# cr1m5onk1ng/text_similarity

Measured on AMD Instinct MI355X. Metric: sentences/sec encoded + Mpairs/sec cosine top-k @ N=1M d=384, higher is better.
Workload: dtype bf16 encoder / f16 selection / fp32 scores

## Files before the change

include/tsim.h:

```cpp
#ifndef TSIM_H
#define TSIM_H

#include <stddef.h>
#include <stdint.h>

#ifdef __cplusplus
extern "C" {
#endif

#define TSIM_OK 0
#define TSIM_EINVAL 1
#define TSIM_EHIP 2
#define TSIM_ENOMEM 3
#define TSIM_EUNSUPPORTED 4

#define TSIM_F32 0
#define TSIM_BF16 1

#define TSIM_ARCH_BERT 0
#define TSIM_ARCH_MPNET 1
#define TSIM_ARCH_ROBERTA 2

int tsim_version(void);
const char *tsim_last_error(void);
// ... 201 lines not shown
    int32_t dense_act;
    int32_t normalize;
} tsim_sentence_head;

int tsim_encoder_forward_head(tsim_encoder *enc, const int32_t *tok_ids, const int32_t *tok_type, const int32_t *tok_pos,
                              const int32_t *tok_col, const int32_t *cu_seqlens, int32_t T, int32_t B, int32_t max_len,
                              const tsim_sentence_head *head, float *emb_f32, void *unit_f16, int ld_unit,
                              float *unit_rho_max, void *last_hidden_bf16, void *stream);

int tsim_encoder_forward_spans(tsim_encoder *enc, const int32_t *tok_ids, const int32_t *tok_type, const int32_t *tok_pos,
                               const int32_t *tok_col, const int32_t *cu_seqlens, int32_t T, int32_t B, int32_t max_len,
                               float *pooled_f32, void *unit_f16, int ld_unit, float *unit_rho_max,
                               void *last_hidden_bf16, float *logits_f32, const int32_t *span_seq, const int32_t *span_cu,
                               const int32_t *span_tok, int32_t S, int32_t n_span_tok, float *span_out_f32,
                               void *span_unit_f16, int ld_span_unit, float *span_rho_max, void *stream);

#define TSIM_ENC_ERR_TOKEN_ID 1
#define TSIM_ENC_ERR_POSITION 2
#define TSIM_ENC_ERR_MAX_LEN 4
#define TSIM_ENC_ERR_TOKEN_TYPE 8
#define TSIM_ENC_ERR_SPAN 16
int tsim_encoder_error_flags(tsim_encoder *enc, int32_t *flags_host, void *stream);

int tsim_wordpiece_create(const char *vocab_text, const int64_t *vocab_offsets, int32_t vocab_size,
                          const char *continuing_prefix, int32_t unk_id, const int32_t *prefix_ids, int32_t n_prefix,
                          const int32_t *suffix_ids, int32_t n_suffix, int32_t lowercase, int32_t max_input_chars_per_word,
                          const char *added_text, const int64_t *added_offsets, int32_t n_added, void **handle);
void tsim_wordpiece_destroy(void *handle);
int tsim_wordpiece_encode(void *handle, const char *text, const int64_t *text_offsets, int64_t n, int32_t max_len,
                          int32_t n_threads, int32_t *out_ids, int64_t out_capacity, int32_t *out_lens, uint8_t *handled);

#ifdef __cplusplus
}
#endif
#endif
```

text_similarity_amd/_lib.py:

```python
from __future__ import annotations

import ctypes as C
import os

_HERE = os.path.dirname(os.path.abspath(__file__))
LIB_PATH = os.environ.get("TSIM_LIB") or os.path.join(_HERE, "libtsim.so")

TSIM_F32, TSIM_BF16 = 0, 1
TSIM_I32, TSIM_I64 = 2, 3
LIST_ST_ROW, LIST_ST_LIMS = 1, 2
ARCH_BERT, ARCH_MPNET, ARCH_ROBERTA = 0, 1, 2
W_BF16, W_MXFP8 = 0, 1
POOL_MEAN, POOL_CLS, POOL_MAX, POOL_MEAN_SQRT_LEN = 0, 1, 2, 3
ACT_IDENTITY, ACT_TANH, ACT_RELU = 0, 1, 2
SPACE_COSINE, SPACE_DOT, SPACE_L2 = 0, 1, 2
ENC_ERR_SPAN = 16
RANGE_SLOT_CAP = 2048
RANGE_MERGE_MAX_LISTS = 64


class TsimError(RuntimeError):
    pass


# ... 104 lines not shown
    "tsim_time_next_topk": (None, [C.c_void_p, C.c_void_p]),
    "tsim_topk_merge": (C.c_int, [C.c_void_p, C.c_void_p, C.c_int, C.c_int64, C.c_int, C.c_int, C.c_void_p,
                                  C.c_void_p, C.c_void_p]),
    "tsim_topk_merge_strided": (C.c_int, [C.c_void_p, C.c_void_p, C.c_int, C.c_int64, C.c_int, C.c_int, C.c_int64, C.c_int64,
                                          C.c_void_p, C.c_void_p, C.c_void_p]),
    "tsim_wordpiece_create": (C.c_int, [C.c_char_p, C.c_void_p, C.c_int32, C.c_char_p, C.c_int32, C.c_void_p, C.c_int32, C.c_void_p,
                                        C.c_int32, C.c_int32, C.c_int32, C.c_char_p, C.c_void_p, C.c_int32, C.POINTER(C.c_void_p)]),
    "tsim_wordpiece_destroy": (None, [C.c_void_p]),
    "tsim_wordpiece_encode": (C.c_int, [C.c_void_p, C.c_char_p, C.c_void_p, C.c_int64, C.c_int32, C.c_int32, C.c_void_p, C.c_int64,
                                        C.c_void_p, C.c_void_p]),
    "tsim_cos_sim": (C.c_int, [C.c_void_p, C.c_int64, C.c_void_p, C.c_int64, C.c_int, C.c_void_p, C.c_void_p]),
    "tsim_mean_pool": (C.c_int, [C.c_void_p, C.c_int, C.c_void_p, C.c_int64, C.c_int, C.c_int, C.c_void_p,
                                 C.c_void_p]),
    "tsim_pool": (C.c_int, [C.c_void_p, C.c_int, C.c_void_p, C.c_int64, C.c_int, C.c_int, C.c_int, C.c_void_p, C.c_void_p]),
    "tsim_dense_rows": (C.c_int, [C.c_void_p, C.c_int64, C.c_int, C.c_void_p, C.c_void_p, C.c_int, C.c_int, C.c_int, C.c_void_p,
                                  C.c_void_p]),
    "tsim_quantize_mxfp8": (C.c_int, [C.c_void_p, C.c_int64, C.c_int, C.c_void_p, C.c_void_p, C.c_void_p]),
    "tsim_gemm_mxfp8": (C.c_int, [C.c_void_p, C.c_void_p, C.c_void_p, C.c_void_p, C.c_void_p, C.c_void_p, C.c_int, C.c_int,
                                  C.c_int, C.c_void_p]),
    "tsim_encoder_create": (C.c_int, [C.POINTER(EncoderConfigC), C.POINTER(EncoderWeightsC),
                                      C.POINTER(C.c_void_p)]),
    "tsim_encoder_destroy": (None, [C.c_void_p]),
    "tsim_encoder_error_flags": (C.c_int, [C.c_void_p, C.POINTER(C.c_int32), C.c_void_p]),
    "tsim_encoder_forward": (C.c_int, [C.c_void_p, C.c_void_p, C.c_void_p, C.c_void_p, C.c_void_p, C.c_int32,
                                       C.c_int32, C.c_int32, C.c_void_p, C.c_void_p, C.c_int, C.c_void_p, C.c_void_p,
                                       C.c_void_p]),
    "tsim_encoder_set_token_types": (C.c_int, [C.c_void_p, C.c_void_p, C.c_int32]),
    "tsim_encoder_set_cls_head": (C.c_int, [C.c_void_p, C.c_void_p, C.c_void_p, C.c_void_p, C.c_void_p, C.c_int32]),
    "tsim_encoder_set_cls_head_act": (C.c_int, [C.c_void_p, C.c_void_p, C.c_void_p, C.c_void_p, C.c_void_p, C.c_int32, C.c_int32]),
    "tsim_encoder_forward_ex": (C.c_int, [C.c_void_p, C.c_void_p, C.c_void_p, C.c_void_p, C.c_void_p, C.c_void_p, C.c_int32,
                                          C.c_int32, C.c_int32, C.c_void_p, C.c_void_p, C.c_int, C.c_void_p, C.c_void_p,
                                          C.c_void_p, C.c_void_p]),
    "tsim_encoder_forward_head": (C.c_int, [C.c_void_p, C.c_void_p, C.c_void_p, C.c_void_p, C.c_void_p, C.c_void_p, C.c_int32,
                                            C.c_int32, C.c_int32, C.POINTER(SentenceHeadC), C.c_void_p, C.c_void_p, C.c_int,
                                            C.c_void_p, C.c_void_p, C.c_void_p]),
    "tsim_encoder_forward_spans": (C.c_int, [C.c_void_p, C.c_void_p, C.c_void_p, C.c_void_p, C.c_void_p, C.c_void_p, C.c_int32,
                                             C.c_int32, C.c_int32, C.c_void_p, C.c_void_p, C.c_int, C.c_void_p, C.c_void_p,
                                             C.c_void_p, C.c_void_p, C.c_void_p, C.c_void_p, C.c_int32, C.c_int32, C.c_void_p,
                                             C.c_void_p, C.c_int, C.c_void_p, C.c_void_p]),
}

DECLARED_SYMBOLS = tuple(_SIGS)


def lib() -> C.CDLL:
    global _lib
# ... 25 lines not shown
```

text_similarity_amd/build.py:

```python
from __future__ import annotations

import os
import subprocess
import sys
from concurrent.futures import ThreadPoolExecutor

HERE = os.path.dirname(os.path.abspath(__file__))
CSRC = os.path.join(HERE, "csrc")
TAG = os.environ.get("TSIM_BUILD_TAG", "")
OBJ = os.path.join(CSRC, "_obj" + ("_" + TAG if TAG else ""))
LIB = os.path.join(HERE, "libtsim" + ("_" + TAG if TAG else "") + ".so")
SOURCES = ["common.hip", "search.hip", "k1_kl16.hip", "k1_d384.hip", "k1_kl32.hip", "k1_collect.hip", "gemm_pp.hip", "encoder.hip",
           "wordpiece.cpp"]
HOT_KERNELS = ("l2_rows_kernel", "l2_query_rows_kernel", "l2_negate_scores", "flag_all_kernel", "cos_topk_partial", "cos_topk_finalize", "gemm_bf16", "gemm_xres", "ln_rows_gemm", "ln_tail_gemm", "gemm_pp", "attention_kernel",
               "pool_packed_kernel", "dense_rows_kernel", "widen_finalize", "bf_partial", "bf_merge",
               "topk_merge_large", "list_prep", "list_partial", "list_merge", "range_setup", "range_finalize", "range_bf", "range_fill", "range_merge", "span_pool_kernel",
               "pack_sign_rows", "hamming_partial", "hamming_merge", "sign_rescore",
               "embed_ln_kernel", "cls_head_kernel", "cls_head_wide_kernel")
FLAGS = ["--offload-arch=gfx950", "-O3", "-std=c++17", "-fPIC", "-fno-gpu-rdc", "-Wall", "-Wno-unused-function",
         "-I" + os.path.join(os.path.dirname(HERE), "include")]


def _newer(a, bs):
    return os.path.exists(a) and all(os.path.getmtime(a) >= os.path.getmtime(b) for b in bs)


DIAGNOSTIC_DEFINES = ("TSIM_LN_DIAG", "TSIM_X2_DIAG", "TSIM_FF_DIAG", "TSIM_K1_NOSEL", "TSIM_PP_STAMPS", "TSIM_K1_DIAG",
                      "TSIM_ATT_DIAG", "TSIM_L_DIAG")


def build(force: bool = False, verbose: bool = True, extra_flags=(), only=None) -> str:
    bad = [f for f in extra_flags if f.startswith("-D") and ("DIAG" in f or any(d in f for d in DIAGNOSTIC_DEFINES))]
    if bad and not TAG:
        raise RuntimeError(f"{bad}: diagnostic defines produce wrong results; they are refused for the product library — "
                           "set TSIM_BUILD_TAG=<tag> to build libtsim_<tag>.so beside it")
    os.makedirs(OBJ, exist_ok=True)
    hdrs = [os.path.join(CSRC, f) for f in os.listdir(CSRC) if f.endswith(".h")]
# ... 65 lines not shown
```

text_similarity_amd/csrc/encoder.hip:

```cpp
#include <math.h>
#include <cmath>

#include <stdlib.h>
#include <string.h>

#include <vector>

#include <type_traits>
#include <utility>

#include "common.h"
#include "gemm_pp.h"

namespace tsim {

__device__ __forceinline__ int64_t packed_off(int64_t t, int f, int W) {
    return ((t >> 5) * (W >> 3) + (f >> 3)) * 256 + (t & 31) * 8 + (f & 7);
}
__device__ __forceinline__ int64_t group_off(int64_t t, int g, int W, int packed) {
    return packed ? packed_off(t, 8 * g, W) * 2 : (t * W + 8 * g) * 2;
}

template <int VPL, bool TYPED = false>
__global__ __launch_bounds__(256) void embed_ln_kernel(const int32_t *__restrict__ ids,
// ... 736 lines not shown
    for (int t = 0; t < 12; ++t) {
        uint32_t pk[8];
#pragma unroll
        for (int gq = 0; gq < 4; ++gq) {
            const int n = 32 * t + 8 * gq + 4 * h;
            const f32x4 gv = *reinterpret_cast<const f32x4 *>(gamma + n), bv = *reinterpret_cast<const f32x4 *>(beta + n);
            const float o0 = fmaf((acc[t][4 * gq + 0] - mean) * rstd, gv[0], bv[0]);
            const float o1 = fmaf((acc[t][4 * gq + 1] - mean) * rstd, gv[1], bv[1]);
            const float o2 = fmaf((acc[t][4 * gq + 2] - mean) * rstd, gv[2], bv[2]);
            const float o3 = fmaf((acc[t][4 * gq + 3] - mean) * rstd, gv[3], bv[3]);
            pk[2 * gq] = pack_bf16x2(o0, o1);
            pk[2 * gq + 1] = pack_bf16x2(o2, o3);
        }
#pragma unroll
        for (int gq = 0; gq < 4; gq += 2) {
            auto s0 = __builtin_amdgcn_permlane32_swap(pk[2 * gq], pk[2 * gq + 2], false, false);
            auto s1w = __builtin_amdgcn_permlane32_swap(pk[2 * gq + 1], pk[2 * gq + 3], false, false);
            if (live)
                *reinterpret_cast<uint4 *>(reinterpret_cast<char *>(out) + (oo + (4 * t + gq) * ogs)) = make_uint4(s0[0], s1w[0], s0[1], s1w[1]);
        }
    }
}

template <int DH, bool REL, bool PK = false>
__global__ __launch_bounds__(256) __attribute__((amdgpu_waves_per_eu(DH <= 32 ? 6 : 4))) void attention_kernel(const bf16_t *__restrict__ qkv,
                                                        const int32_t *__restrict__ cu, const int32_t *__restrict__ col,
                                                        const float *__restrict__ relb, int relw, int H,
                                                        int heads, float scale, bf16_t *__restrict__ ctx, int B, int xcd_map) {
    constexpr int KS = DH / 16;
    constexpr int OT = (DH + 31) / 32;
    constexpr int ROWB = DH * 2 < 64 ? 64 : DH * 2;
    __shared__ __attribute__((aligned(16))) char vimg[4 * 32 * ROWB];
    typedef __attribute__((ext_vector_type(4))) short s16x4;
    const int lane = threadIdx.x & 63;
    const int wave = __builtin_amdgcn_readfirstlane(threadIdx.x >> 6);
    int seq = blockIdx.x;
    if (xcd_map) {
        seq = (blockIdx.x & 7) * (gridDim.x >> 3) + (blockIdx.x >> 3);
        if (seq >= B) return;
    }
    const int head = blockIdx.y * 4 + wave, qb = blockIdx.z;
    const int t0 = cu[seq], S = cu[seq + 1] - t0;
    if (qb * 32 >= S || head >= heads) return;
    const int r = lane & 31, h = lane >> 5;
    const int64_t H3 = 3 * (int64_t)H;
    const int qi = qb * 32 + r;
// ... 902 lines not shown
                           K, xpacked ? 1 : 0, rpk);
    TSIM_HIP_CHECK(hipGetLastError());
    hipLaunchKernelGGL(ln_split_finish_kernel, dim3((unsigned)nb), dim3(256), 0, st, im, gamma, beta, eps, out, M, opk);
    TSIM_HIP_CHECK(hipGetLastError());
    return TSIM_OK;
}

template <int NW, int NST>
static int ln_rows_gemm(const bf16_t *X, const bf16_t *Wimg32, const float *bias, const bf16_t *res, const float *gamma,
                        const float *beta, float eps, bf16_t *out, int M, int K, hipStream_t st, bool xpacked, bool respacked, bool opacked) {
    constexpr int lds = NST * (NW * 32 * LR_BK * 2 + LR_WBYTES);
    static_assert(lds <= 160 * 1024, "LDS budget");
    auto kern = ln_rows_gemm_kernel<NW, NST>;
    static DevOnce lds_once;
    TSIM_MAX_LDS(lds_once, kern, lds);
    if (K % LR_BK != 0 || K < NST * LR_BK) return fail(TSIM_EUNSUPPORTED, "ln_rows_gemm: K=%d", K);
    if (((int64_t)M + 256) * 768 >= (1ll << 32)) return fail(TSIM_EUNSUPPORTED, "ln_rows_gemm: %d rows of 384 exceed 4 GiB", M);
    hipLaunchKernelGGL(kern, dim3((unsigned)((M + NW * 32 - 1) / (NW * 32))), dim3(NW * 64), lds, st, X, Wimg32, bias, res, gamma,
                       beta, eps, out, M, K, xpacked ? 1 : 0, respacked ? 1 : 0, opacked ? 1 : 0);
    TSIM_HIP_CHECK(hipGetLastError());
    return TSIM_OK;
}

static bool use_packed_layout(int H, int F) {
    return H == 384 && (3 * H) % X2_BN == 0 && F % X2_BN == 0 && F <= 2048;
}

template <int EPI>
static int gemm_plain(const bf16_t *X, const bf16_t *W, const bf16_t *Wp, const float *bias, bf16_t *out, int M, int N,
                      int K, hipStream_t st) {
    if (K == 384 && N % XR_BN == 0) return gemm_xres2<EPI, false>(X, W, bias, out, M, N, st);
    if (K >= 768 && gemm_pp_supported(N, K))
        return gemm_pp(EPI == EPI_GELU ? PP_EPI_GELU : PP_EPI_BIAS, X, Wp ? Wp : W, Wp != nullptr, bias, out, M, N, K, st);
    if (N % 128 == 0)
        return launch_gemm<128, 128, 64, 2, 2, EPI>(X, W, bias, nullptr, nullptr, nullptr, 0.f, out, M, N, K, st);
    return launch_gemm<128, 64, 64, 2, 2, EPI>(X, W, bias, nullptr, nullptr, nullptr, 0.f, out, M, N, K, st);
}

static int gemm_res_ln(const bf16_t *X, const bf16_t *W, const bf16_t *Wp, const float *bias, const bf16_t *res,
                       const float *gamma, const float *beta, float eps, bf16_t *out, int M, int N, int K, float *ybuf,
                       hipStream_t st, const bf16_t *Wimg = nullptr, const bf16_t *Wimg32 = nullptr, bool xpacked = false,
                       float *lnimg = nullptr, bool respacked = false, bool opacked = false) {
    if ((xpacked || respacked || opacked) && N != 384) return fail(TSIM_EINVAL, "gemm_res_ln: the packed layouts are a hidden-384 form");
    if (ybuf && N >= 512 && N % 256 == 0 && gemm_pp_supported(N, K)) {
        int rc = gemm_pp(PP_EPI_F32, X, Wp ? Wp : W, Wp != nullptr, bias, ybuf, M, N, K, st);
        if (rc) return rc;
        return res_ln_rows(ybuf, res, gamma, beta, eps, out, nullptr, nullptr, M, N, st);
    }
    switch (N) {
        case 384: {
            bool after_rows = false;
            if (Wimg32) {
                const int t256 = M / 256;
                const int use = (t256 % 256) >= 128 ? t256 : (t256 / 256) * 256;
                if (use > 0) {
                    int rc = ln_rows_gemm<8, 3>(X, Wimg32, bias, res, gamma, beta, eps, out, use * 256, K, st, xpacked, respacked, opacked);
                    const int m1 = use * 256;
                    if (rc || m1 == M) return rc;
                    X += (int64_t)m1 * K; res += (int64_t)m1 * N; out += (int64_t)m1 * N; M -= m1;
                    after_rows = true;
                }
                if (M <= LS_MAX_BLOCKS * 32 && K % (16 * LT_PF) == 0)
                    return ln_tail_gemm(X, Wimg32, bias, res, gamma, beta, eps, out, M, K, st, xpacked, lnimg, respacked, opacked);
            }
            const int mt = (M + 127) / 128, full = (mt / 256) * 256, rem = mt - full;
            auto main_launch = [&](int rows) {
                return launch_gemm<128, 384, 64, 2, 4, EPI_RES_LN>(X, W, bias, res, gamma, beta, eps, out, rows, N, K, st, Wimg, xpacked, respacked, opacked);
            };
            if (rem > 0 && rem <= 96 && (full > 0 || after_rows)) {
                const int m_main = full * 128;
                if (full > 0) {
                    int rc = main_launch(m_main);
                    if (rc) return rc;
                }
                return launch_gemm<64, 384, 64, 2, 4, EPI_RES_LN>(X + (int64_t)m_main * K, W, bias, res + (int64_t)m_main * N,
                                                                  gamma, beta, eps, out + (int64_t)m_main * N, M - m_main, N, K, st, Wimg, xpacked, respacked, opacked);
            }
            return main_launch(M);
        }
        case 768: return launch_gemm<64, 768, 32, 1, 8, EPI_RES_LN>(X, W, bias, res, gamma, beta, eps, out, M, N, K, st);
        case 64: return launch_gemm<128, 64, 64, 4, 2, EPI_RES_LN>(X, W, bias, res, gamma, beta, eps, out, M, N, K, st);
        default: return fail(TSIM_EUNSUPPORTED, "encoder: hidden size %d has no fused LayerNorm GEMM (64, 384, 768)", N);
    }
}

}

extern "C" int tsim_encoder_create(const tsim_encoder_config *cfg, const tsim_encoder_weights_host *w,
                                   tsim_encoder **out) {
    TSIM_REQUIRE(cfg && w && out, "encoder_create: null pointer");
    const int H = cfg->hidden, F = cfg->ffn, L = cfg->num_layers;
    TSIM_REQUIRE(H == 64 || H == 384 || H == 768 || H == 1024, "encoder_create: hidden=%d unsupported (64, 384, 768, 1024)", H);
    TSIM_REQUIRE(cfg->heads > 0 && H % cfg->heads == 0, "encoder_create: heads=%d does not divide hidden=%d", cfg->heads, H);
    const int dh = H / cfg->heads;
    TSIM_REQUIRE(dh == 16 || dh == 32 || dh == 64, "encoder_create: head_dim=%d unsupported (16, 32, 64)", dh);
    TSIM_REQUIRE(F % 64 == 0 && L > 0 && cfg->max_tokens > 0 && cfg->max_seqs > 0, "encoder_create: bad ffn/layers/capacity");
    TSIM_REQUIRE(cfg->arch == TSIM_ARCH_BERT || cfg->arch == TSIM_ARCH_MPNET || cfg->arch == TSIM_ARCH_ROBERTA, "encoder_create: unknown arch");
    TSIM_REQUIRE(w->word_emb && w->pos_emb && w->emb_ln_g && w->emb_ln_b && w->layers, "encoder_create: missing weights");
    TSIM_REQUIRE(cfg->arch != TSIM_ARCH_MPNET || w->rel_bias, "encoder_create: MPNet needs rel_bias");
    const bool mx = cfg->weight_dtype == TSIM_W_MXFP8;
    TSIM_REQUIRE(cfg->weight_dtype == TSIM_W_BF16 || mx, "encoder_create: unknown weight_dtype %d", cfg->weight_dtype);
    if (mx && !(gemm_pp_mx_supported(H, H) && gemm_pp_mx_supported(3 * H, H) && gemm_pp_mx_supported(F, H) && gemm_pp_mx_supported(H, F)))
        return fail(TSIM_EUNSUPPORTED, "encoder_create: MXFP8 projections need hidden and ffn to be multiples of 256 (got %d, %d)", H, F);
    tsim_encoder *e = new tsim_encoder();
    e->cfg = *cfg;
    e->Tp = (cfg->max_tokens + 127) / 128 * 128 + 128;
    int rc = TSIM_OK;
    auto bail = [&](int code) {
// ... 210 lines not shown
    hipStream_t st = reinterpret_cast<hipStream_t>(stream);
    const tsim_encoder_config &c = e->cfg;
    const int H = c.hidden, F = c.ffn, dh = H / c.heads;
    const bool mx = c.weight_dtype == TSIM_W_MXFP8;
    int rc;
    if (T > 0) {
        const unsigned g = (unsigned)((T + 3) / 4);
        const int32_t *colp = tok_col ? tok_col : tok_pos;
        const int col_limit = tok_col || c.arch == TSIM_ARCH_BERT ? max_len : c.max_pos;
#define EMBED(V) hipLaunchKernelGGL(embed_ln_kernel<V>, dim3(g), dim3(256), 0, st, tok_ids, tok_pos, e->word, e->pos, e->type0, e->emb_g, e->emb_b, c.ln_eps, T, H, e->x0, c.vocab, c.max_pos, colp, col_limit, e->err_flags, nullptr, 0)
#define EMBED_T(V) hipLaunchKernelGGL((embed_ln_kernel<V, true>), dim3(g), dim3(256), 0, st, tok_ids, tok_pos, e->word, e->pos, e->type0, e->emb_g, e->emb_b, c.ln_eps, T, H, e->x0, c.vocab, c.max_pos, colp, col_limit, e->err_flags, tok_type, e->n_types)
        if (tok_type) {
            if (H == 64) EMBED_T(1); else if (H == 384) EMBED_T(6); else if (H == 768) EMBED_T(12); else EMBED_T(16);
        } else if (H == 64) EMBED(1); else if (H == 384) EMBED(6); else if (H == 768) EMBED(12); else EMBED(16);
#undef EMBED_T
#undef EMBED
        TSIM_HIP_CHECK(hipGetLastError());
        const float scale = 1.0f / sqrtf((float)dh);
        const bool rel = c.arch == TSIM_ARCH_MPNET;
        const bool pk = !mx && !rel && use_packed_layout(H, F);
        const int32_t *col = rel ? (tok_col ? tok_col : tok_pos) : nullptr;
        const int qblocks = (max_len + 31) / 32 > 0 ? (max_len + 31) / 32 : 1;
        const dim3 agrid((unsigned)(((B + 7) / 8) * 8), (unsigned)((c.heads + 3) / 4), (unsigned)qblocks);
        for (int l = 0; l < c.num_layers; ++l) {
            const tsim_encoder::Layer &L = e->layers[l];
            const bool x0pk = pk && l > 0, x0pk_next = pk && l + 1 < c.num_layers;
            if (mx) {
                if (l == 0 && (rc = quant_mx(e->x0, T, H, e->aq, e->as, st))) return rc;
                if ((rc = gemm_pp_mx(PP_EPI_BIAS, e->aq, e->as, L.qqkv, 1, L.sqkv, L.bqkv, e->qkv, nullptr, T, 3 * H, H, st))) return rc;
            } else if (pk) {
                rc = x0pk ? gemm_xres2<EPI_BIAS, true, true>(e->x0, L.wqkv, L.bqkv, e->qkv, T, 3 * H, st)
                          : gemm_xres2<EPI_BIAS, true>(e->x0, L.wqkv, L.bqkv, e->qkv, T, 3 * H, st);
                if (rc) return rc;
            } else if ((rc = gemm_plain<EPI_BIAS>(e->x0, L.wqkv, L.pqkv, L.bqkv, e->qkv, T, 3 * H, H, st))) return rc;
#define ATT(D)                                                                                                 \
    do {                                                                                                       \
        if (rel)                                                                                               \
            hipLaunchKernelGGL((attention_kernel<D, true>), agrid, dim3(256), 0, st, e->qkv, cu_seqlens, col,  \
                               e->relb, e->relw, H, c.heads, scale, e->ctx, B, 1);                                         \
        else if (pk)                                                                                           \
            hipLaunchKernelGGL((attention_kernel<D, false, true>), agrid, dim3(256), 0, st, e->qkv, cu_seqlens, col, \
                               e->relb, e->relw, H, c.heads, scale, e->ctx, B, 1);                                         \
        else                                                                                                   \
            hipLaunchKernelGGL((attention_kernel<D, false>), agrid, dim3(256), 0, st, e->qkv, cu_seqlens, col, \
                               e->relb, e->relw, H, c.heads, scale, e->ctx, B, 1);                                         \
    } while (0)
            if (dh == 16) ATT(16); else if (dh == 32) ATT(32); else ATT(64);
#undef ATT
            TSIM_HIP_CHECK(hipGetLastError());
            if (mx) {
                if ((rc = quant_mx(e->ctx, T, H, e->aq, e->as, st))) return rc;
                if ((rc = gemm_pp_mx(PP_EPI_F32, e->aq, e->as, L.qo, 1, L.so, L.bo, e->ybuf, nullptr, T, H, H, st))) return rc;
                if ((rc = res_ln_rows(e->ybuf, e->x0, L.g1, L.be1, c.ln_eps, e->x1, e->aq, e->as, T, H, st))) return rc;
                if ((rc = gemm_pp_mx(PP_EPI_GELU_MX, e->aq, e->as, L.q1, 1, L.s1, L.b1, e->hq, e->hs, T, F, H, st))) return rc;
                if ((rc = gemm_pp_mx(PP_EPI_F32, e->hq, e->hs, L.q2, 1, L.s2, L.b2, e->ybuf, nullptr, T, H, F, st))) return rc;
                if ((rc = res_ln_rows(e->ybuf, e->x1, L.g2, L.be2, c.ln_eps, e->x0, e->aq, e->as, T, H, st))) return rc;
                continue;
            }
            if ((rc = gemm_res_ln(e->ctx, L.wo, L.po, L.bo, e->x0, L.g1, L.be1, c.ln_eps, e->x1, T, H, H, e->ybuf, st, L.lo, L.lo32, false, e->lnimg, x0pk, pk))) return rc;
            if (pk) {
                if ((rc = gemm_xres2<EPI_GELU, true, true>(e->x1, L.w1, L.b1, e->h1, T, F, st))) return rc;
            } else if ((rc = gemm_plain<EPI_GELU>(e->x1, L.w1, nullptr, L.b1, e->h1, T, F, H, st))) return rc;
            if ((rc = gemm_res_ln(e->h1, L.w2, nullptr, L.b2, e->x1, L.g2, L.be2, c.ln_eps, e->x0, T, H, F, e->ybuf, st, L.l2, L.l232, pk, e->lnimg, pk, x0pk_next))) return rc;
        }
        if (last_hidden_bf16)
            TSIM_HIP_CHECK(hipMemcpyAsync(last_hidden_bf16, e->x0, (size_t)T * H * 2, hipMemcpyDeviceToDevice, st));
    }
    if (pooled_f32 || unit_bf16) {
        const unsigned g = (unsigned)((B + 3) / 4);
#define POOL(V) hipLaunchKernelGGL(pool_packed_kernel<V>, dim3(g), dim3(256), 0, st, e->x0, cu_seqlens, B, H, pooled_f32, (unit_t *)unit_bf16, ld_unit, unit_bf16 ? unit_rho_max : nullptr)
        if (H % 8 != 0 || H > 1024 || (unit_bf16 && ld_unit % 8 != 0))
            return fail(TSIM_EUNSUPPORTED, "encoder: pooling needs a hidden size that is a multiple of 8, at most 1024 (got %d)", H);
        if (((uintptr_t)pooled_f32 | (uintptr_t)unit_bf16) & 15)
            return fail(TSIM_EINVAL, "encoder: pooled / unit outputs must be 16-byte aligned");
        if (H <= 512) POOL(1); else POOL(2);
#undef POOL
        TSIM_HIP_CHECK(hipGetLastError());
    }
    if (logits_f32) {
        const dim3 cgrid((unsigned)((B + CLS_ROWS - 1) / CLS_ROWS)), cblock((unsigned)H);
#define CLS_WIDE(MAXH, ACT)                                                                                       \
    hipLaunchKernelGGL((cls_head_wide_kernel<MAXH, ACT>), cgrid, cblock, 0, st, e->x0, cu_seqlens, B, H, e->head_wpT, \
                       e->head_bp, e->head_wc, e->head_bc, e->n_labels, logits_f32)
        if (e->head_act == TSIM_ACT_RELU) {
            if (H <= CLS_MAX_H) CLS_WIDE(CLS_MAX_H, TSIM_ACT_RELU); else CLS_WIDE(CLS_WIDE_H, TSIM_ACT_RELU);
        } else if (H <= CLS_MAX_H) {
// ... 69 lines not shown
```

Baseline: 856,200.

## Fuse residual-LayerNorm GEMM with following FFN-up / next-layer QKV GEMM in one kernel

```diff
diff --git a/include/tsim.h b/include/tsim.h
--- a/include/tsim.h
+++ b/include/tsim.h
@@ -247,6 +247,8 @@
 #define TSIM_ENC_ERR_SPAN 16
 int tsim_encoder_error_flags(tsim_encoder *enc, int32_t *flags_host, void *stream);
 
+int tsim_chain_items_host(int blocks, int rem_blocks, int ntiles, int G, int b, int32_t *items, int cap);
+
 int tsim_wordpiece_create(const char *vocab_text, const int64_t *vocab_offsets, int32_t vocab_size,
                           const char *continuing_prefix, int32_t unk_id, const int32_t *prefix_ids, int32_t n_prefix,
                           const int32_t *suffix_ids, int32_t n_suffix, int32_t lowercase, int32_t max_input_chars_per_word,
diff --git a/text_similarity_amd/_lib.py b/text_similarity_amd/_lib.py
--- a/text_similarity_amd/_lib.py
+++ b/text_similarity_amd/_lib.py
@@ -150,6 +150,7 @@
                                       C.POINTER(C.c_void_p)]),
     "tsim_encoder_destroy": (None, [C.c_void_p]),
     "tsim_encoder_error_flags": (C.c_int, [C.c_void_p, C.POINTER(C.c_int32), C.c_void_p]),
+    "tsim_chain_items_host": (C.c_int, [C.c_int, C.c_int, C.c_int, C.c_int, C.c_int, C.POINTER(C.c_int32), C.c_int]),
     "tsim_encoder_forward": (C.c_int, [C.c_void_p, C.c_void_p, C.c_void_p, C.c_void_p, C.c_void_p, C.c_int32,
                                        C.c_int32, C.c_int32, C.c_void_p, C.c_void_p, C.c_int, C.c_void_p, C.c_void_p,
                                        C.c_void_p]),
diff --git a/text_similarity_amd/build.py b/text_similarity_amd/build.py
--- a/text_similarity_amd/build.py
+++ b/text_similarity_amd/build.py
@@ -12,7 +12,7 @@
 LIB = os.path.join(HERE, "libtsim" + ("_" + TAG if TAG else "") + ".so")
 SOURCES = ["common.hip", "search.hip", "k1_kl16.hip", "k1_d384.hip", "k1_kl32.hip", "k1_collect.hip", "gemm_pp.hip", "encoder.hip",
            "wordpiece.cpp"]
-HOT_KERNELS = ("l2_rows_kernel", "l2_query_rows_kernel", "l2_negate_scores", "flag_all_kernel", "cos_topk_partial", "cos_topk_finalize", "gemm_bf16", "gemm_xres", "ln_rows_gemm", "ln_tail_gemm", "gemm_pp", "attention_kernel",
+HOT_KERNELS = ("l2_rows_kernel", "l2_query_rows_kernel", "l2_negate_scores", "flag_all_kernel", "cos_topk_partial", "cos_topk_finalize", "gemm_bf16", "gemm_xres", "ln_rows_gemm", "ln_rows_xres2", "ln_tail_gemm", "gemm_pp", "attention_kernel",
                "pool_packed_kernel", "dense_rows_kernel", "widen_finalize", "bf_partial", "bf_merge",
                "topk_merge_large", "list_prep", "list_partial", "list_merge", "range_setup", "range_finalize", "range_bf", "range_fill", "range_merge", "span_pool_kernel",
                "pack_sign_rows", "hamming_partial", "hamming_merge", "sign_rescore",
diff --git a/text_similarity_amd/csrc/encoder.hip b/text_similarity_amd/csrc/encoder.hip
--- a/text_similarity_amd/csrc/encoder.hip
+++ b/text_similarity_amd/csrc/encoder.hip
@@ -782,6 +782,380 @@
     }
 }
 
+struct ChainPart { int own, r0, n; };
+__host__ __device__ inline ChainPart chain_part(int G, int rem_blocks, int ntiles, int b) {
+    const long long R = (long long)rem_blocks * ntiles;
+    const int r0 = (int)(R * b / G), r1 = (int)(R * (b + 1) / G);
+    return {ntiles, r0, ntiles + r1 - r0};
+}
+__host__ __device__ inline int chain_item(const ChainPart &p, int G, int ntiles, int b, int i) {
+    return i < p.own ? b * ntiles + i : G * ntiles + p.r0 + (i - p.own);
+}
+
+template <int EPI>
+__global__ __launch_bounds__(512) void ln_rows_xres2_kernel(const bf16_t *__restrict__ X, const bf16_t *__restrict__ Wimg,
+                                                            const float *__restrict__ lbias, const bf16_t *__restrict__ res,
+                                                            const float *__restrict__ gamma, const float *__restrict__ beta,
+                                                            float eps, bf16_t *xout, int K, int xpacked, int respacked,
+                                                            const bf16_t *__restrict__ W2, const float *__restrict__ bias2,
+                                                            bf16_t *__restrict__ out2, int M, int N2, int rem_blocks) {
+    constexpr int NW = 8, N = 384, LR_NST = 3;
+    constexpr int XBYTES = NW * 32 * LR_BK * 2, LSTAGE = XBYTES + LR_WBYTES;
+    constexpr int XP = XBYTES / 1024, LPPW = LSTAGE / 1024 / NW;
+    constexpr int KSTEPS = N / 16, BMX = NW * 32;
+    constexpr int STAGE = X2_BN * X2_BK * 2, PPW = STAGE / 1024 / NW;
+    constexpr int BIAS_OFF = X2_NSTAGE * STAGE, GB_OFF = BIAS_OFF + 6144;
+    static_assert(LR_NST * LSTAGE <= BIAS_OFF && XP == 2 * NW && PPW == 3 && 2 * PPW + 24 <= 63, "hand-over layout");
+    extern __shared__ __attribute__((aligned(16))) char smem[];
+    const int lane = threadIdx.x & 63;
+    const int wave = __builtin_amdgcn_readfirstlane(threadIdx.x >> 6);
+    const int r = lane & 31, h = lane >> 5;
+    const int m0l = blockIdx.x * BMX;
+    const int nk = K / LR_BK;
+    const uint32_t lbase = (uint32_t)(uintptr_t)((__attribute__((address_space(3))) char *)smem);
+
+    for (int p = wave; p * 256 < N2; p += NW)
+        if (p * 256 + lane * 4 < N2) glds16(bias2 + p * 256 + lane * 4, smem + BIAS_OFF + p * 1024);
+    if (wave < 2 && wave * 256 + lane * 4 < N) {
+        glds16(gamma + wave * 256 + lane * 4, smem + GB_OFF + wave * 1024);
+        glds16(beta + wave * 256 + lane * 4, smem + GB_OFF + N * 4 + wave * 1024);
+    }
+
+    f32x16 acc[12];
+#pragma unroll
+    for (int t = 0; t < 12; ++t)
+#pragma unroll
+        for (int gq = 0; gq < 4; ++gq) {
+            const f32x4 bv = *reinterpret_cast<const f32x4 *>(lbias + 32 * t + 8 * gq + 4 * h);
+#pragma unroll
+            for (int e = 0; e < 4; ++e) acc[t][4 * gq + e] = bv[e];
+        }
+    {
+        const char *xsrc[2];
+#pragma unroll
+        for (int i = 0; i < 2; ++i) {
+            const int sl = (wave + i * NW) * 64 + lane;
+            const int sr = sl >> 4, ch = (sl & 15) ^ (sr & 15);
+            const int64_t m = m0l + sr * 4 + (ch >> 2);
+            xsrc[i] = xpacked ? reinterpret_cast<const char *>(X + packed_off(m, (ch & 3) * 8, K))
+                              : reinterpret_cast<const char *>(X) + m * K * 2 + (ch & 3) * 16;
+        }
+        const int xkstride = xpacked ? (LR_BK / 8) * 512 : LR_BK * 2;
+        const char *wsrc = reinterpret_cast<const char *>(Wimg) + lane * 16;
+        auto issue = [&](int kt, int stage) __attribute__((always_inline)) {
+            const int k2 = kt < nk ? kt : nk - 1;
+            char *dst = smem + stage * LSTAGE;
+#pragma unroll
+            for (int i = 0; i < 2; ++i) glds16(xsrc[i] + k2 * xkstride, dst + (wave + i * NW) * 1024);
+#pragma unroll
+            for (int i = 2; i < LPPW; ++i)
+                glds16(wsrc + (int64_t)k2 * LR_WBYTES + (wave + i * NW - XP) * 1024, dst + (wave + i * NW) * 1024);
+        };
+        uint32_t xo[2];
+#pragma unroll
+        for (int sk = 0; sk < 2; ++sk) {
+            const int ch = (r & 3) * 4 + 2 * sk + h;
+            xo[sk] = lbase + wave * 2048 + (r >> 2) * 256 + ((ch ^ ((((wave & 1) << 3) + (r >> 2)) & 15)) << 4);
+        }
+        const uint32_t wl = lbase + XBYTES + lane * 16;
+#pragma unroll
+        for (int i = 0; i < LR_NST - 1; ++i) issue(i, i);
+#pragma unroll
+        for (int t = 0; t < 12; ++t) asm volatile("" : "+v"(acc[t]));
+        auto do_tile = [&](int kt, auto stc) __attribute__((always_inline)) {
+            constexpr int stage = decltype(stc)::value;
+            wait_vmcnt<(LR_NST - 2) * LPPW>();
+            __builtin_amdgcn_s_barrier();
+            issue(kt + LR_NST - 1, (stage + LR_NST - 1) % LR_NST);
+            constexpr int PF = 4, NRD = 24;
+            lds_u32x4 bfr[2], fr[PF + 1];
+            const uint32_t so = stage * LSTAGE;
+            lds_read_b128_imm<0>(bfr[0], xo[0] + so);
+            lds_read_b128_imm<0>(bfr[1], xo[1] + so);
+            const uint32_t wa = wl + so;
+            auto rd = [&](auto nc) __attribute__((always_inline)) {
+                constexpr int n = decltype(nc)::value;
+                lds_read_b128_imm<n * 1024>(fr[n % (PF + 1)], wa);
+            };
+            ff_static_for(std::make_integer_sequence<int, PF>{}, rd);
+            ff_static_for(std::make_integer_sequence<int, NRD>{}, [&](auto nc) __attribute__((always_inline)) {
+                constexpr int n = decltype(nc)::value;
+                if constexpr (n + PF < NRD) rd(std::integral_constant<int, n + PF>{});
+                constexpr int younger = n + PF < NRD ? PF : NRD - 1 - n;
+                lgkm_wait_counted<younger>(fr[n % (PF + 1)]);
+                if constexpr (n == 0) { asm volatile("" : "+v"(bfr[0])); asm volatile("" : "+v"(bfr[1])); }
+                acc[n % 12] = __builtin_amdgcn_mfma_f32_32x32x16_bf16(__builtin_bit_cast(bf16x8, fr[n % (PF + 1)]),
+                                                                       __builtin_bit_cast(bf16x8, bfr[n / 12]), acc[n % 12], 0, 0, 0);
+            });
+        };
+        int kt = 0;
+        for (; kt + LR_NST <= nk; kt += LR_NST)
+            ff_static_for(std::make_integer_sequence<int, LR_NST>{}, [&](auto sc) __attribute__((always_inline)) {
+                do_tile(kt + decltype(sc)::value, sc);
+            });
+        ff_static_for(std::make_integer_sequence<int, LR_NST - 1>{}, [&](auto sc) __attribute__((always_inline)) {
+            if (kt + decltype(sc)::value < nk) do_tile(kt + decltype(sc)::value, sc);
+        });
+    }
+    wait_vmcnt<0>();
+    __builtin_amdgcn_s_barrier();
+
+    const int ntiles = N2 / X2_BN, G = (int)gridDim.x, wg = (int)blockIdx.x;
+    const ChainPart part = chain_part(G, rem_blocks, ntiles, wg);
+    auto w_src_off = [&](int ln, int i) __attribute__((always_inline)) {
+        const int sl = (wave * PPW + i) * 64 + ln;
+        const int row = sl >> 4, ch = (sl & 15) ^ (row & 15);
+        return row * N * 2 + ch * 16;
+    };
+    int pi = 0, pg = 0, pj = chain_item(part, G, ntiles, wg, 0) % ntiles;
+    auto tile_base = [&]() __attribute__((always_inline)) {
+        return reinterpret_cast<const char *>(W2) + ((int64_t)pj * X2_BN * N + pg * X2_BK) * 2;
+    };
+    auto advance = [&]() __attribute__((always_inline)) {
+        if (++pg == X2_KG) {
+            if (pi + 1 < part.n) {
+                pg = 0;
+                ++pi;
+                pj = chain_item(part, G, ntiles, wg, pi) % ntiles;
+            } else {
+                pg = X2_KG - 1;
+            }
+        }
+    };
+    const int lanep = __builtin_amdgcn_mbcnt_hi(~0u, __builtin_amdgcn_mbcnt_lo(~0u, 0u));
+#pragma unroll
+    for (int i = 0; i < X2_PD; ++i) {
+        const char *base = tile_base();
+#pragma unroll
+        for (int p = 0; p < PPW; ++p) glds16(base + w_src_off(lanep, p), smem + i * STAGE + (wave * PPW + p) * 1024);
+        advance();
+    }
+
+    bf16x8 bx[KSTEPS];
+    {
+        const int lane1 = __builtin_amdgcn_mbcnt_hi(~0u, __builtin_amdgcn_mbcnt_lo(~0u, 0u));
+        const uint32_t ro = (uint32_t)group_off(m0l + wave * 32 + (lane1 & 31), lane1 >> 5, N, respacked), rgs = (uint32_t)group_off(0, 1, N, respacked);
+#pragma unroll
+        for (int t = 0; t < 12; ++t)
+#pragma unroll
+            for (int gq = 0; gq < 4; gq += 2) {
+                const uint4 o = *reinterpret_cast<const uint4 *>(reinterpret_cast<const char *>(res) + (ro + (4 * t + gq) * rgs));
+                auto s0 = __builtin_amdgcn_permlane32_swap(o.x, o.z, false, false);
+                auto s1 = __builtin_amdgcn_permlane32_swap(o.y, o.w, false, false);
+                const uint32_t a0 = s0[0], c0 = s0[1], a1 = s1[0], c1 = s1[1];
+                acc[t][4 * gq + 0] += __uint_as_float(a0 << 16);
+                acc[t][4 * gq + 1] += __uint_as_float(a0 & 0xffff0000u);
+                acc[t][4 * gq + 2] += __uint_as_float(a1 << 16);
+                acc[t][4 * gq + 3] += __uint_as_float(a1 & 0xffff0000u);
+                acc[t][4 * gq + 4] += __uint_as_float(c0 << 16);
+                acc[t][4 * gq + 5] += __uint_as_float(c0 & 0xffff0000u);
+                acc[t][4 * gq + 6] += __uint_as_float(c1 << 16);
+                acc[t][4 * gq + 7] += __uint_as_float(c1 & 0xffff0000u);
+            }
+        float mean, rstd;
+#pragma unroll
+        for (int pass = 0; pass < 2; ++pass) {
+            float tot = 0.f;
+#pragma unroll
+            for (int w = 0; w < 4; ++w) {
+                float sg = 0.f;
+#pragma unroll
+                for (int t = 3 * w; t < 3 * w + 3; ++t)
+#pragma unroll
+                    for (int q = 0; q < 16; ++q) {
+                        if (pass == 0) {
+                            sg += acc[t][q];
+                        } else {
+                            const float dlt = acc[t][q] - mean;
+                            sg = fmaf(dlt, dlt, sg);
+                        }
+                    }
+                sg += __shfl_xor(sg, 32, 64);
+                tot += sg;
+            }
+            if (pass == 0)
+                mean = tot / (float)N;
+            else
+                rstd = 1.0f / sqrtf(tot / (float)N + eps);
+        }
+        int lane3 = __builtin_amdgcn_mbcnt_hi(~0u, __builtin_amdgcn_mbcnt_lo(~0u, 0u));
+        asm volatile("" : "+v"(lane3));
+        const int h3 = lane3 >> 5;
+        const uint32_t oo = (uint32_t)group_off(m0l + wave * 32 + (lane3 & 31), h3, N, 1);
+        constexpr uint32_t ogs = 512;
+        const uint64_t xb = (uint64_t)(uintptr_t)xout;
+        const float *gl = reinterpret_cast<const float *>(smem + GB_OFF), *bl = gl + N;
+#pragma unroll
+        for (int t = 0; t < 12; ++t) {
+            uint32_t pk[8];
+#pragma unroll
+            for (int gq = 0; gq < 4; ++gq) {
+                const int n = 32 * t + 8 * gq + 4 * h3;
+                const f32x4 gv = *reinterpret_cast<const f32x4 *>(gl + n), bv = *reinterpret_cast<const f32x4 *>(bl + n);
+                const float o0 = fmaf((acc[t][4 * gq + 0] - mean) * rstd, gv[0], bv[0]);
+                const float o1 = fmaf((acc[t][4 * gq + 1] - mean) * rstd, gv[1], bv[1]);
+                const float o2 = fmaf((acc[t][4 * gq + 2] - mean) * rstd, gv[2], bv[2]);
+                const float o3 = fmaf((acc[t][4 * gq + 3] - mean) * rstd, gv[3], bv[3]);
+                pk[2 * gq] = pack_bf16x2(o0, o1);
+                pk[2 * gq + 1] = pack_bf16x2(o2, o3);
+            }
+#pragma unroll
+            for (int gq = 0; gq < 4; gq += 2) {
+                auto s0 = __builtin_amdgcn_permlane32_swap(pk[2 * gq], pk[2 * gq + 2], false, false);
+                auto s1w = __builtin_amdgcn_permlane32_swap(pk[2 * gq + 1], pk[2 * gq + 3], false, false);
+                const u32x4 o = {s0[0], s1w[0], s0[1], s1w[1]};
+                const uint32_t voff = oo + (4 * t + gq) * ogs;
+                asm volatile("global_store_dwordx4 %0, %1, %2\n\ts_nop 1" ::"v"(voff), "v"(o), "s"(xb) : "memory");
+                bx[2 * t + gq / 2] = __builtin_bit_cast(bf16x8, o);
+            }
+        }
+    }
+
+    int lane2 = __builtin_amdgcn_mbcnt_hi(~0u, __builtin_amdgcn_mbcnt_lo(~0u, 0u));
+    asm volatile("" : "+v"(lane2));
+    const int r2 = lane2 & 31, h2 = lane2 >> 5;
+    int src_off[PPW];
+#pragma unroll
+    for (int i = 0; i < PPW; ++i) src_off[i] = w_src_off(lane2, i);
+    auto issue_pieces = [&](int stage, int i0, int i1) __attribute__((always_inline)) {
+        const char *base = tile_base();
+        for (int i = i0; i < i1; ++i)
+            glds16(base + src_off[i], smem + stage * STAGE + (wave * PPW + i) * 1024);
+    };
+    int cks[8];
+#pragma unroll
+    for (int ks = 0; ks < 8; ++ks) cks[ks] = r2 * 256 + (((2 * ks + h2) ^ (r2 & 15)) << 4);
+    const uint32_t bias_lds = lbase + BIAS_OFF;
+    int cur_mb = wg, m0 = wg * BMX + wave * 32;
+    f32x16 accA[X2_NSUB], accB[X2_NSUB];
+    int old_m0 = 0, old_n0 = 0;
+    int st = 0, ring = 0;
+    int young1 = 0, young2 = 0, young3 = 0;
+    int carry = 1;
+    uint32_t old_rowoff = 0;
+    const uint64_t out_base = (uint64_t)(uintptr_t)out2;
+    auto store_half = [&](const uint32_t (&pk)[8], int mrow0, int ncol, auto gqc) __attribute__((always_inline)) {
+        constexpr int gq = decltype(gqc)::value;
+        const bool full = mrow0 + 32 <= M;
+        uint32_t a0 = pk[2 * gq], a1 = pk[2 * gq + 1], b0 = pk[2 * gq + 2], b1 = pk[2 * gq + 3];
+        auto s0 = __builtin_amdgcn_permlane32_swap(a0, b0, false, false);
+        auto s1 = __builtin_amdgcn_permlane32_swap(a1, b1, false, false);
+        const u32x4 o = {s0[0], s1[0], s0[1], s1[1]};
+        const uint32_t voff = old_rowoff + (uint32_t)(ncol + 8 * gq) * 64u;
+        const uint64_t ob = out_base;
+        if (full || mrow0 + r2 < M)
+            asm volatile("global_store_dwordx4 %0, %1, %2\n\ts_nop 1" ::"v"(voff), "v"(o), "s"(ob) : "memory");
+    };
+    auto finish2 = [&](float y0, float y1) __attribute__((always_inline)) -> uint32_t {
+        if constexpr (EPI == EPI_GELU) gelu2(y0, y1);
+        return pack_bf16x2(y0, y1);
+    };
+    auto run_item = [&](f32x16 (&cur)[X2_NSUB], f32x16 (&old)[X2_NSUB], int item, auto with_old) __attribute__((always_inline)) {
+        constexpr bool OLD = decltype(with_old)::value;
+        const int gi = chain_item(part, G, ntiles, wg, item);
+        if (gi / ntiles != cur_mb) {
+            cur_mb = gi / ntiles;
+            m0 = cur_mb * BMX + wave * 32;
+            const char *xp = reinterpret_cast<const char *>(xout) + group_off(m0 + r2, h2, N, 1);
+#pragma unroll
+            for (int s = 0; s < KSTEPS; ++s) bx[s] = *reinterpret_cast<const bf16x8 *>(xp + 2 * s * 512);
+#pragma unroll
+            for (int s = 0; s < KSTEPS; ++s) asm volatile("" : "+v"(bx[s]));
+            young1 = young2 = young3 = 0;
+            carry = 0;
+        }
+        const int n0 = (gi % ntiles) * X2_BN;
+        const uint32_t baddr = bias_lds + (n0 + 4 * h2) * 4;
+        ff_static_for(std::make_integer_sequence<int, X2_NSUB>{}, [&](auto ic) __attribute__((always_inline)) {
+            constexpr int i = decltype(ic)::value;
+            f32x4 bv[4];
+            asm volatile("ds_read_b128 %0, %1 offset:%2" : "=v"(bv[0]) : "v"(baddr), "n"((i * 32 + 0) * 4) : "memory");
+            asm volatile("ds_read_b128 %0, %1 offset:%2" : "=v"(bv[1]) : "v"(baddr), "n"((i * 32 + 8) * 4) : "memory");
+            asm volatile("ds_read_b128 %0, %1 offset:%2" : "=v"(bv[2]) : "v"(baddr), "n"((i * 32 + 16) * 4) : "memory");
+            asm volatile("ds_read_b128 %0, %1 offset:%2" : "=v"(bv[3]) : "v"(baddr), "n"((i * 32 + 24) * 4) : "memory");
+            asm volatile("s_waitcnt lgkmcnt(0)" : "+v"(bv[0]), "+v"(bv[1]), "+v"(bv[2]), "+v"(bv[3])::"memory");
+#pragma unroll
+            for (int q = 0; q < 16; ++q) cur[i][q] = bv[q >> 2][q & 3];
+        });
+#pragma unroll
+        for (int g = 0; g < X2_KG; ++g) {
+            asm volatile("" : "+s"(ring));
+            const int stage = ring;
+            if ((st & 1) == 0) {
+                const int ys = (young1 >= 0 && young2 >= 0 && young3 >= 0) ? young1 + young2 + young3 : 0;
+                if (carry) wait_vmcnt<2 * PPW + 24>();
+                else if (ys == 6) wait_vmcnt<2 * PPW + 6>();
+                else if (ys == 4) wait_vmcnt<2 * PPW + 4>();
+                else if (ys == 2) wait_vmcnt<2 * PPW + 2>();
+                else wait_vmcnt<2 * PPW>();
+                __builtin_amdgcn_s_barrier();
+            }
+            __builtin_amdgcn_sched_barrier(0);
+            uint32_t pk[8];
+            {
+                constexpr int PF = 3, NRD = 8 * X2_NSUB;
+                lds_u32x4 fr[PF + 1];
+                const uint32_t wsl = lbase + stage * STAGE;
+                auto rd = [&](auto nc) __attribute__((always_inline)) {
+                    constexpr int n = decltype(nc)::value;
+                    lds_read_b128_imm<(n % X2_NSUB) * 8192>(fr[n % (PF + 1)], wsl + cks[n / X2_NSUB]);
+                };
+                ff_static_for(std::make_integer_sequence<int, PF>{}, rd);
+                ff_static_for(std::make_integer_sequence<int, NRD>{}, [&](auto nc) __attribute__((always_inline)) {
+                    constexpr int n = decltype(nc)::value;
+                    constexpr int ks = n / X2_NSUB, i = n % X2_NSUB;
+                    if constexpr (n + PF < NRD) rd(std::integral_constant<int, n + PF>{});
+                    constexpr int younger = n + PF < NRD ? PF : NRD - 1 - n;
+                    lgkm_wait_counted<younger>(fr[n % (PF + 1)]);
+                    cur[i] = __builtin_amdgcn_mfma_f32_32x32x16_bf16(__builtin_bit_cast(bf16x8, fr[n % (PF + 1)]), bx[g * 8 + ks], cur[i], 0, 0, 0);
+                    if constexpr (i == X2_NSUB - 1) {
+                        if constexpr (ks == 1 || ks == 3 || ks == 5) {
+                            const int ns = stage + X2_PD;
+                            issue_pieces(ns >= X2_NSTAGE ? ns - X2_NSTAGE : ns, ks >> 1, (ks >> 1) + 1);
+                            if constexpr (ks == 5) advance();
+                        }
+                        if constexpr (OLD) pk[ks] = finish2(old[g][2 * ks], old[g][2 * ks + 1]);
+                    }
+                });
+            }
+            young3 = young2;
+            young2 = young1;
+            young1 = 0;
+            if constexpr (OLD) {
+                store_half(pk, old_m0, old_n0 + g * 32, std::integral_constant<int, 0>{});
+                store_half(pk, old_m0, old_n0 + g * 32, std::integral_constant<int, 2>{});
+                young1 = old_m0 + 32 <= M ? 2 : -1;
+            }
+            ++st;
+            ring = ring + 1 == X2_NSTAGE ? 0 : ring + 1;
+            if (st >= 3) carry = 0;
+        }
+        old_m0 = m0;
+        old_n0 = n0;
+        old_rowoff = (uint32_t)(m0 >> 5) * (uint32_t)(N2 * 64) + 16u * r2 + 512u * h2;
+    };
+    int item = 0;
+    run_item(accA, accB, item++, std::false_type{});
+    for (; item + 2 <= part.n; item += 2) {
+        run_item(accB, accA, item, std::true_type{});
+        run_item(accA, accB, item + 1, std::true_type{});
+    }
+    const bool lastA = item >= part.n;
+    if (!lastA) run_item(accB, accA, item, std::true_type{});
+    wait_vmcnt<0>();
+    auto flush = [&](f32x16 (&a)[X2_NSUB]) __attribute__((always_inline)) {
+#pragma unroll
+        for (int g = 0; g < X2_NSUB; ++g) {
+            uint32_t pk[8];
+#pragma unroll
+            for (int ks = 0; ks < 8; ++ks) pk[ks] = finish2(a[g][2 * ks], a[g][2 * ks + 1]);
+            store_half(pk, old_m0, old_n0 + g * 32, std::integral_constant<int, 0>{});
+            store_half(pk, old_m0, old_n0 + g * 32, std::integral_constant<int, 2>{});
+        }
+    };
+    if (lastA) flush(accA); else flush(accB);
+}
+
 template <int DH, bool REL, bool PK = false>
 __global__ __launch_bounds__(256) __attribute__((amdgpu_waves_per_eu(DH <= 32 ? 6 : 4))) void attention_kernel(const bf16_t *__restrict__ qkv,
                                                         const int32_t *__restrict__ cu, const int32_t *__restrict__ col,
@@ -1730,6 +2104,32 @@
     return TSIM_OK;
 }
 
+static int ln_rows_blocks(int M) {
+    const int t256 = M / 256;
+    return (t256 % 256) >= 128 ? t256 : (t256 / 256) * 256;
+}
+
+template <int EPI>
+static int ln_rows_xres2(const bf16_t *X, const bf16_t *Wimg32, const float *lbias, const bf16_t *res, const float *gamma,
+                         const float *beta, float eps, bf16_t *xout, int blocks, int K, bool xpacked, bool respacked, const bf16_t *W2,
+                         const float *bias2, bf16_t *out2, int M, int N2, hipStream_t st) {
+    constexpr int lds = X2_NSTAGE * X2_BN * X2_BK * 2 + 6144 + 2 * 384 * 4;
+    static_assert(lds <= 160 * 1024, "LDS budget");
+    if (N2 % X2_BN != 0 || N2 > 1536) return fail(TSIM_EUNSUPPORTED, "ln_rows_xres2: N=%d", N2);
+    if (K % LR_BK != 0 || K < 3 * LR_BK) return fail(TSIM_EUNSUPPORTED, "ln_rows_xres2: K=%d", K);
+    if (blocks <= 0 || (int64_t)blocks * 256 > M) return fail(TSIM_EINVAL, "ln_rows_xres2: %d blocks of %d rows", blocks, M);
+    if (((int64_t)M + 256) * N2 * 2 >= (1ll << 32) || ((int64_t)M + 256) * 768 >= (1ll << 32))
+        return fail(TSIM_EUNSUPPORTED, "ln_rows_xres2: output of %d x %d exceeds 4 GiB", M, N2);
+    auto kern = ln_rows_xres2_kernel<EPI>;
+    static DevOnce lds_once;
+    TSIM_MAX_LDS(lds_once, kern, lds);
+    const int rem_blocks = (M - blocks * 256 + 255) / 256;
+    hipLaunchKernelGGL(kern, dim3((unsigned)blocks), dim3(512), lds, st, X, Wimg32, lbias, res, gamma, beta, eps, xout, K,
+                       xpacked ? 1 : 0, respacked ? 1 : 0, W2, bias2, out2, M, N2, rem_blocks);
+    TSIM_HIP_CHECK(hipGetLastError());
+    return TSIM_OK;
+}
+
 static bool use_packed_layout(int H, int F) {
     return H == 384 && (3 * H) % X2_BN == 0 && F % X2_BN == 0 && F <= 2048;
 }
@@ -1748,7 +2148,7 @@
 static int gemm_res_ln(const bf16_t *X, const bf16_t *W, const bf16_t *Wp, const float *bias, const bf16_t *res,
                        const float *gamma, const float *beta, float eps, bf16_t *out, int M, int N, int K, float *ybuf,
                        hipStream_t st, const bf16_t *Wimg = nullptr, const bf16_t *Wimg32 = nullptr, bool xpacked = false,
-                       float *lnimg = nullptr, bool respacked = false, bool opacked = false) {
+                       float *lnimg = nullptr, bool respacked = false, bool opacked = false, bool tail_only = false) {
     if ((xpacked || respacked || opacked) && N != 384) return fail(TSIM_EINVAL, "gemm_res_ln: the packed layouts are a hidden-384 form");
     if (ybuf && N >= 512 && N % 256 == 0 && gemm_pp_supported(N, K)) {
         int rc = gemm_pp(PP_EPI_F32, X, Wp ? Wp : W, Wp != nullptr, bias, ybuf, M, N, K, st);
@@ -1759,10 +2159,10 @@
         case 384: {
             bool after_rows = false;
             if (Wimg32) {
-                const int t256 = M / 256;
-                const int use = (t256 % 256) >= 128 ? t256 : (t256 / 256) * 256;
+                const int use = ln_rows_blocks(M);
                 if (use > 0) {
-                    int rc = ln_rows_gemm<8, 3>(X, Wimg32, bias, res, gamma, beta, eps, out, use * 256, K, st, xpacked, respacked, opacked);
+                    int rc = tail_only ? TSIM_OK
+                                       : ln_rows_gemm<8, 3>(X, Wimg32, bias, res, gamma, beta, eps, out, use * 256, K, st, xpacked, respacked, opacked);
                     const int m1 = use * 256;
                     if (rc || m1 == M) return rc;
                     X += (int64_t)m1 * K; res += (int64_t)m1 * N; out += (int64_t)m1 * N; M -= m1;
@@ -1792,6 +2192,13 @@
     }
 }
 
+}
+
+extern "C" int tsim_chain_items_host(int blocks, int rem_blocks, int ntiles, int G, int b, int32_t *items, int cap) {
+    if (blocks != G || rem_blocks < 0 || ntiles <= 0 || G <= 0 || b < 0 || b >= G || (cap > 0 && !items)) return -1;
+    const ChainPart p = chain_part(G, rem_blocks, ntiles, b);
+    for (int i = 0; i < p.n && i < cap; ++i) items[i] = chain_item(p, G, ntiles, b, i);
+    return p.n;
 }
 
 extern "C" int tsim_encoder_create(const tsim_encoder_config *cfg, const tsim_encoder_weights_host *w,
@@ -2048,6 +2455,7 @@
         const int32_t *col = rel ? (tok_col ? tok_col : tok_pos) : nullptr;
         const int qblocks = (max_len + 31) / 32 > 0 ? (max_len + 31) / 32 : 1;
         const dim3 agrid((unsigned)(((B + 7) / 8) * 8), (unsigned)((c.heads + 3) / 4), (unsigned)qblocks);
+        bool qkv_chained = false;
         for (int l = 0; l < c.num_layers; ++l) {
             const tsim_encoder::Layer &L = e->layers[l];
             const bool x0pk = pk && l > 0, x0pk_next = pk && l + 1 < c.num_layers;
@@ -2055,9 +2463,11 @@
                 if (l == 0 && (rc = quant_mx(e->x0, T, H, e->aq, e->as, st))) return rc;
                 if ((rc = gemm_pp_mx(PP_EPI_BIAS, e->aq, e->as, L.qqkv, 1, L.sqkv, L.bqkv, e->qkv, nullptr, T, 3 * H, H, st))) return rc;
             } else if (pk) {
-                rc = x0pk ? gemm_xres2<EPI_BIAS, true, true>(e->x0, L.wqkv, L.bqkv, e->qkv, T, 3 * H, st)
-                          : gemm_xres2<EPI_BIAS, true>(e->x0, L.wqkv, L.bqkv, e->qkv, T, 3 * H, st);
-                if (rc) return rc;
+                if (!qkv_chained) {
+                    rc = x0pk ? gemm_xres2<EPI_BIAS, true, true>(e->x0, L.wqkv, L.bqkv, e->qkv, T, 3 * H, st)
+                              : gemm_xres2<EPI_BIAS, true>(e->x0, L.wqkv, L.bqkv, e->qkv, T, 3 * H, st);
+                    if (rc) return rc;
+                }
             } else if ((rc = gemm_plain<EPI_BIAS>(e->x0, L.wqkv, L.pqkv, L.bqkv, e->qkv, T, 3 * H, H, st))) return rc;
 #define ATT(D)                                                                                                 \
     do {                                                                                                       \
@@ -2083,11 +2493,24 @@
                 if ((rc = res_ln_rows(e->ybuf, e->x1, L.g2, L.be2, c.ln_eps, e->x0, e->aq, e->as, T, H, st))) return rc;
                 continue;
             }
-            if ((rc = gemm_res_ln(e->ctx, L.wo, L.po, L.bo, e->x0, L.g1, L.be1, c.ln_eps, e->x1, T, H, H, e->ybuf, st, L.lo, L.lo32, false, e->lnimg, x0pk, pk))) return rc;
-            if (pk) {
-                if ((rc = gemm_xres2<EPI_GELU, true, true>(e->x1, L.w1, L.b1, e->h1, T, F, st))) return rc;
-            } else if ((rc = gemm_plain<EPI_GELU>(e->x1, L.w1, nullptr, L.b1, e->h1, T, F, H, st))) return rc;
-            if ((rc = gemm_res_ln(e->h1, L.w2, nullptr, L.b2, e->x1, L.g2, L.be2, c.ln_eps, e->x0, T, H, F, e->ybuf, st, L.l2, L.l232, pk, e->lnimg, pk, x0pk_next))) return rc;
+            const int chain_blocks = pk && F <= 1536 && ln_rows_blocks(T) % 256 == 0 ? ln_rows_blocks(T) : 0;
+            if (chain_blocks > 0 && L.lo32) {
+                if ((rc = gemm_res_ln(e->ctx, L.wo, L.po, L.bo, e->x0, L.g1, L.be1, c.ln_eps, e->x1, T, H, H, e->ybuf, st, L.lo, L.lo32, false, e->lnimg, x0pk, pk, true))) return rc;
+                if ((rc = ln_rows_xres2<EPI_GELU>(e->ctx, L.lo32, L.bo, e->x0, L.g1, L.be1, c.ln_eps, e->x1, chain_blocks, H, false, x0pk,
+                                                  L.w1, L.b1, e->h1, T, F, st))) return rc;
+            } else {
+                if ((rc = gemm_res_ln(e->ctx, L.wo, L.po, L.bo, e->x0, L.g1, L.be1, c.ln_eps, e->x1, T, H, H, e->ybuf, st, L.lo, L.lo32, false, e->lnimg, x0pk, pk))) return rc;
+                if (pk) {
+                    if ((rc = gemm_xres2<EPI_GELU, true, true>(e->x1, L.w1, L.b1, e->h1, T, F, st))) return rc;
+                } else if ((rc = gemm_plain<EPI_GELU>(e->x1, L.w1, nullptr, L.b1, e->h1, T, F, H, st))) return rc;
+            }
+            qkv_chained = chain_blocks > 0 && L.l232 && x0pk_next;
+            if (qkv_chained) {
+                const tsim_encoder::Layer &Ln = e->layers[l + 1];
+                if ((rc = gemm_res_ln(e->h1, L.w2, nullptr, L.b2, e->x1, L.g2, L.be2, c.ln_eps, e->x0, T, H, F, e->ybuf, st, L.l2, L.l232, pk, e->lnimg, pk, true, true))) return rc;
+                if ((rc = ln_rows_xres2<EPI_BIAS>(e->h1, L.l232, L.b2, e->x1, L.g2, L.be2, c.ln_eps, e->x0, chain_blocks, F, true, true,
+                                                  Ln.wqkv, Ln.bqkv, e->qkv, T, 3 * H, st))) return rc;
+            } else if ((rc = gemm_res_ln(e->h1, L.w2, nullptr, L.b2, e->x1, L.g2, L.be2, c.ln_eps, e->x0, T, H, F, e->ybuf, st, L.l2, L.l232, pk, e->lnimg, pk, x0pk_next))) return rc;
         }
         if (last_hidden_bf16)
             TSIM_HIP_CHECK(hipMemcpyAsync(last_hidden_bf16, e->x0, (size_t)T * H * 2, hipMemcpyDeviceToDevice, st));
```

Result: faster. 888,600, median of 6 (+3.8%).
